# daihangpku/SW-NeRF

Hardware: AMD Instinct MI355X
Metric: rays/sec (64+128 samples/ray) (higher is better)
Workload: dtype f32

## Files before the change

### sw-nerf_amd/csrc/colour_kernels.hip

```cpp
#include <hip/hip_runtime.h>
#include "../../include/swnerf.h"
#include "swnerf_common.h"
#include "mlp_core.h"
#include "host_util.h"
#include "mlp_kernels.h"
#include "render_pass.h"

__global__ void __launch_bounds__(1024) colour_scan_kernel(ViewWs vw, int64_t n_rays) {
    __shared__ int part[16];
    const int tid = threadIdx.x, lane = tid & 63, wv = tid >> 6;
    const int64_t K = (n_rays + 1023) / 1024;
    const int64_t r0 = tid * K, r1 = r0 + K < n_rays ? r0 + K : n_rays;
    int* off = vw_off(vw);
    int* segray = vw_segray(vw, n_rays);
    int sum = 0;
    for (int64_t r = r0; r < r1; ++r) sum += off[r];
    int v = sum;
#pragma unroll
    for (int o = 1; o < 64; o <<= 1) { const int up = __shfl_up(v, o, 64); if (lane >= o) v += up; }
    if (lane == 63) part[wv] = v;
    __syncthreads();
    int below = v - sum, total = 0;
#pragma unroll
    for (int k = 0; k < 16; ++k) { if (k < wv) below += part[k]; total += part[k]; }
    for (int64_t r = r0; r < r1; ++r) {
        const int cnt = off[r];
        off[r] = below;
        for (int g = (below + 31) >> 5; 32 * g < below + cnt; ++g) segray[g] = (int)r;
        below += cnt;
    }
    if (tid == 0) off[n_rays] = total;
}

struct ColourDev {
    ViewWs vw;
    const float* ray_batch; int cols; int64_t n_rays;
    const float* b0; int nbias;
    const float* wvl;
};

__global__ void __launch_bounds__(256, 2) colour_rows_kernel(ColourDev P) {
    extern __shared__ __attribute__((aligned(16))) float lds_bias[];
    const int lane = threadIdx.x & 63, j = lane & 31, h = lane >> 5;
    const int wv = __builtin_amdgcn_readfirstlane(threadIdx.x >> 6);
    bias_to_lds(lds_bias, P.b0, P.nbias);
    const int* off = vw_off(P.vw);
    const int* segray = vw_segray(P.vw, P.n_rays);
    const int total = __builtin_amdgcn_readfirstlane(off[P.n_rays]);
    const int nseg = (total + 31) >> 5, nwaves = (int)gridDim.x * 4;
    int g = (int)blockIdx.x * 4 + wv;
    if (g >= nseg) return;
    WStream ws;
    ws_start(ws, P.wvl, lds_bias, lds_bias + P.nbias + wv * SW_RING * SW_STEP_FLOATS, lane);
    const float* rgb_tiles = ws.bias + (SW_DIR_BIAS_TILES + 64 + 8 + 1) * SW_BIAS_TILE_FLOATS;
    const float* hb_rgb = rgb_tiles - SW_BIAS_TILE_FLOATS;
    const int gs = vw_group_stride(P.vw);
#pragma nounroll
    for (; g < nseg; g += nwaves) {
        const int row = 32 * g + j;
        const bool valid = row < total;
        const int i = valid ? row : total - 1;
        const int rg = __builtin_amdgcn_readfirstlane(segray[g]);
        const int64_t rk = (int64_t)rg + j + 1;
        const int nxt = off[rk < P.n_rays ? rk : P.n_rays];
        int dr = 0;
#pragma unroll
        for (int k = 0; k < 32; ++k) dr += (__shfl(nxt, k, 32) <= i) ? 1 : 0;
        const int64_t ray = (int64_t)rg + dr;
        const int slot = i - off[ray];
        float* reg = vw_ray(P.vw, ray);
        const int s = vw_sample(P.vw, reg)[slot];
        const float* q = vw_row(P.vw, reg, slot, h);
        f32x16 in[8], demb, hv[4];
#pragma unroll
        for (int c = 0; c < 32; ++c) {
            const f32x4 v = *reinterpret_cast<const f32x4*>(q + (size_t)c * gs);
            in[c >> 2][4 * (c & 3) + 0] = v[0]; in[c >> 2][4 * (c & 3) + 1] = v[1];
            in[c >> 2][4 * (c & 3) + 2] = v[2]; in[c >> 2][4 * (c & 3) + 3] = v[3];
        }
        const float* dp = P.ray_batch + ray * P.cols + (P.cols - 3);
        pe_dir(dp[0], dp[1], dp[2], h, demb);
        ws.bias = rgb_tiles;
        ws.base = reinterpret_cast<const char*>(P.wvl);
        canon_tail_rows(in, demb, hv, lds_bias + h * 16, ws);
        float c3[3];
        head_valu<3, 4>(hv, ws, c3);
        if (valid && h == 0) {
            float* c = vw_c(P.vw, reg);
            c[s] = c3[0] + hb_rgb[1]; c[P.vw.sp + s] = c3[1] + hb_rgb[2]; c[2 * P.vw.sp + s] = c3[2] + hb_rgb[3];
        }
    }
}

__global__ void __launch_bounds__(256) colour_maps_kernel(ViewWs vw, int64_t n_rays, int S, int white, float* rgb_map) {
    const int lane = threadIdx.x & 63, j = lane & 31;
    const int64_t ray = (int64_t)blockIdx.x * 4 + (threadIdx.x >> 6);
    if (ray >= n_rays) return;
    float* reg = vw_ray(vw, ray);
    const float* wq = vw_w(vw, reg);
    const float* cq = vw_c(vw, reg);
    float pr = 0.f, pg = 0.f, pb = 0.f;
    const int ntiles = (S + 31) >> 5;
#pragma nounroll
    for (int t = 0; t < ntiles; ++t) {
        const int s = t * 32 + j;
        const int sc = s < S ? s : S - 1;
        const float w = s < S ? wq[sc] : 0.f;
        const float c0 = cq[sc], c1 = cq[vw.sp + sc], c2 = cq[2 * vw.sp + sc];
        comp_accumulate_colour(w, c0, c1, c2, pr, pg, pb);
    }
    pr = wave32_sum(pr); pg = wave32_sum(pg); pb = wave32_sum(pb);
    if (lane == 0) comp_write_rgb(pr, pg, pb, reg[0], white, ray, rgb_map);
}

int sw_colour_split_launch(const swnerf_pass_args& a, const ViewWs& vw, const float* b0, int nbias, const float* wvl, hipStream_t st) {
    hipLaunchKernelGGL(colour_scan_kernel, dim3(1), dim3(1024), 0, st, vw, a.n_rays);
    const int64_t rows_max = a.n_rays * (int64_t)(vw.rows < a.n_samples ? vw.rows : a.n_samples);
    const int64_t wgs = (rows_max + 127) / 128;
    if (wgs > 0) {
        ColourDev P;
        P.vw = vw; P.ray_batch = a.ray_batch; P.cols = a.cols; P.n_rays = a.n_rays; P.b0 = b0; P.nbias = nbias; P.wvl = wvl;
        const size_t lds = ((size_t)nbias + 4 * SW_RING * SW_STEP_FLOATS) * sizeof(float);
        hipLaunchKernelGGL(colour_rows_kernel, dim3((unsigned)(wgs < 512 ? wgs : 512)), dim3(256), lds, st, P);
    }
    hipLaunchKernelGGL(colour_maps_kernel, dim3((unsigned)((a.n_rays + 3) / 4)), dim3(256), 0, st, vw, a.n_rays, a.n_samples, a.white_bkgd, a.rgb_map);
    return sw_check(hipGetLastError(), "render_pass colour launch");
}
```

### sw-nerf_amd/csrc/render_pass.h

```cpp
#pragma once
#include <cstdlib>
#include "mlp_kernels.h"
#include "mlp_core_x3.h"
#include "resample.h"
#include "composite.h"
#include "ray_rows.h"

#define SW_LDS_SC 256
#define SW_LDS_SORT 1024
#define SW_LDS_WAVE_FLOATS (3 * SW_LDS_SC + SW_LDS_SORT)

#define SW_DEFER_SMAX 240
#define SW_DEFER_WS_FLOATS (64 * 256)
#define SW_DEFER_SEGS_PER_RAY ((SW_DEFER_SMAX + 31) / 32)

struct ViewWs {
    float* base;
    int64_t hdr, per_ray;
    int rows, sp;
};

static inline int64_t view_ws_hdr(int64_t n_rays) { return ((n_rays + 1 + 3) & ~(int64_t)3) + SW_DEFER_SEGS_PER_RAY * n_rays; }
static inline int64_t view_ws_full(int64_t n_rays, int S) {
    const int64_t sp = (S + 3) & ~3;
    return view_ws_hdr(n_rays) + n_rays * (4 + 4 * sp + 257 * sp);
}
static inline ViewWs view_ws_layout(float* base, int64_t floats, int64_t n_rays, int S) {
    ViewWs v = {};
    v.base = base;
    v.sp = (S + 3) & ~3;
    v.hdr = view_ws_hdr(n_rays);
    const int64_t avail = n_rays > 0 ? ((floats - v.hdr) / n_rays) & ~(int64_t)3 : 0;
    int64_t r = ((avail - 4 - 4 * v.sp) / 257) & ~(int64_t)3;
    if (r > v.sp) r = v.sp;
    v.rows = r > 0 ? (int)r : 0;
    v.per_ray = 4 + 4 * (int64_t)v.sp + 257 * (int64_t)v.rows;
    return v;
}
__device__ __forceinline__ int* vw_off(const ViewWs& v) { return reinterpret_cast<int*>(v.base); }
__device__ __forceinline__ int* vw_segray(const ViewWs& v, int64_t n_rays) { return reinterpret_cast<int*>(v.base) + ((n_rays + 1 + 3) & ~(int64_t)3); }
__device__ __forceinline__ float* vw_ray(const ViewWs& v, int64_t ray) { return v.base + v.hdr + ray * v.per_ray; }
__device__ __forceinline__ float* vw_w(const ViewWs& v, float* reg) { return reg + 4; }
__device__ __forceinline__ float* vw_c(const ViewWs& v, float* reg) { return reg + 4 + v.sp; }
__device__ __forceinline__ int* vw_sample(const ViewWs& v, float* reg) { return reinterpret_cast<int*>(reg + 4 + 4 * v.sp); }
__device__ __forceinline__ float* vw_row(const ViewWs& v, float* reg, int slot, int h) { return reg + 4 + 4 * v.sp + v.rows + (h * v.rows + slot) * 4; }
__device__ __forceinline__ int vw_group_stride(const ViewWs& v) { return 8 * v.rows; }

struct PassDev {
    swnerf_pass_args a;
    const float* w0;
    const float* b0;
    int nbias;
    int two_pass;
    int sort_n, sort_s;
    float* act;
    float* bits;
    float* xs;
    float* act_d; float* bits_d; float* xs_d;
    int dir_steps;
    int time_steps;
    int tb_off;
    int warm_steps;
    int warm_blocks;
    int skew_mode;
    int skew_unit;
    ViewWs vw;
};

__device__ __forceinline__ float wave32_sum(float v) {
#pragma unroll
    for (int o = 16; o > 0; o >>= 1) v += __shfl_xor(v, o, 32);
    return v;
}

__device__ __forceinline__ float z_linear(const swnerf_pass_args& a, float near, float far, int s) {
    const float t = sw_linspace(0.f, 1.f, a.n_samples, s);
    if (!a.lindisp) return near * (1.f - t) + far * t;
    return 1.f / (1.f / near * (1.f - t) + 1.f / far * t);
}

__device__ __forceinline__ float z_sample(const swnerf_pass_args& a, int64_t ray, float near, float far, int s) {
    const int S = a.n_samples;
    if (a.z_vals) return a.z_vals[ray * S + s];
    const float zs = z_linear(a, near, far, s);
    if (!a.t_rand) return zs;
    const float upper = (s < S - 1) ? .5f * (z_linear(a, near, far, s + 1) + zs) : zs;
    const float lower = (s > 0) ? .5f * (zs + z_linear(a, near, far, s - 1)) : zs;
    return lower + (upper - lower) * a.t_rand[ray * S + s];
}

#define SW_WARM_MAX_PER_WAVE 48
__device__ __forceinline__ void pass_startup(const PassDev& P, const float* w0, float* junk, int lane, int wv) {
    const unsigned b = blockIdx.x;
    if (P.warm_steps > 0 && (int)(b >> 3) < P.warm_blocks) {
        const unsigned junk_addr = __builtin_amdgcn_readfirstlane((unsigned)(size_t)junk);
        const int stride = P.warm_blocks * 4;
        int s = (int)(b >> 3) * 4 + wv;
#pragma nounroll
        for (int i = 0; i < SW_WARM_MAX_PER_WAVE && s < P.warm_steps; ++i, s += stride)
            ws_dma(reinterpret_cast<const char*>(w0) + (size_t)s * 1024, (unsigned)lane * 16u, junk_addr);
    }
    if (P.skew_mode) {
        const int k = (P.skew_mode == 1 ? (int)(b >> 3) : (int)(b >> 3) * 4 + wv) & 15;
#pragma nounroll
        for (int i = 0; i < k; ++i) __builtin_amdgcn_s_sleep(4);
        (void)P.skew_unit;
    }
}

static inline void pass_startup_args(PassDev& P, unsigned grid_x, int steps) {
    const char* ew = getenv("SWNERF_WARM");
    const char* es = getenv("SWNERF_SKEW");
    const int env_warm = ew ? atoi(ew) : 1, env_skew = es ? atoi(es) : 2;
    const unsigned first_round = grid_x < 256u ? grid_x : 256u;
    P.warm_blocks = (int)(first_round / 8u);
    P.warm_steps = (env_warm && P.warm_blocks > 0) ? steps + SW_TAIL : 0;
    P.skew_mode = env_skew;
    P.skew_unit = 4;
}

struct PassAccepts {
    const char* name;
    unsigned cols[4];
    int shape_code;
    const char* shape_msg;
    bool time_band;
    int smax;
};
#define SW_COLS(c) (1u << (c))

static inline int pass_check(const PassAccepts& e, const swnerf_pass_args& a) {
    if (!a.packed || (!a.ray_batch && a.n_rays != 0)) return sw_fail(SWNERF_E_ARG, e.smax ? "%s: NULL pointer" : "%s: NULL ray_batch/packed", e.name);
    if (a.kind < 0 || a.kind > 3 || a.cols < 0 || a.cols > 31 || !(e.cols[a.kind] >> a.cols & 1u)) return sw_fail(e.shape_code, e.shape_msg, e.name, a.cols, a.kind);
    if (e.smax && (a.n_rays < 0 || a.n_samples < 2 || a.n_samples > e.smax))
        return sw_fail(SWNERF_E_UNSUPP, "%s: 2 <= n_samples <= %d (got %d)", e.name, e.smax, a.n_samples);
    if (a.n_rays < 0 || a.n_samples < 2) return sw_fail(SWNERF_E_ARG, "%s: n_rays %lld, n_samples %d", e.name, (long long)a.n_rays, a.n_samples);
    if (a.L_pos < 0 || a.L_pos > 10 || a.L_dir < 0 || a.L_dir > 4 || (e.time_band && (a.L_time < 0 || a.L_time > 10)))
        return e.time_band ? sw_fail(SWNERF_E_UNSUPP, "%s: embedder bands (%d,%d,%d) exceed (10,4,10)", e.name, a.L_pos, a.L_dir, a.L_time)
                           : sw_fail(SWNERF_E_UNSUPP, "%s: embedder bands (%d,%d) exceed (10,4)", e.name, a.L_pos, a.L_dir);
    if (a.z_vals && a.t_rand) return sw_fail(SWNERF_E_ARG, "%s: t_rand only applies to coarse sampling", e.name);
    return 0;
}

static inline PassDev pass_dev(const swnerf_pass_args& a) {
    PassDev P = {};
    P.a = a;
    return P;
}

static inline int pass_resampling(const char* name, const swnerf_pass_args& a, PassDev& P, size_t& lds) {
    if (a.n_importance <= 0) return 0;
    if (!a.z_fine && a.n_rays != 0) return sw_fail(SWNERF_E_ARG, "%s: n_importance>0 needs z_fine", name);
    if (a.n_samples < 3 || a.n_samples > SW_LDS_SC || a.n_samples + a.n_importance > SW_LDS_SORT)
        return sw_fail(SWNERF_E_UNSUPP, "%s: resampling supports 3<=N_samples<=%d and N_samples+N_importance<=%d", name, SW_LDS_SC, SW_LDS_SORT);
    P.sort_n = P.sort_s = 2;
    while (P.sort_n < a.n_importance) P.sort_n <<= 1;
    while (P.sort_s < a.n_samples) P.sort_s <<= 1;
    lds += 4 * SW_LDS_WAVE_FLOATS * sizeof(float);
    return 0;
}

template <bool VEC4>
__device__ __forceinline__ void comp_bwd_ray(const float* raw, int oc, const float* zv, const float* noise, int S, int lane, float dnorm,
                                             int white, const float* g_rgb, const float* g_disp, const float* g_acc,
                                             float* T_, float* W_, float* dR) {
    CompGrads g = {g_rgb ? g_rgb[0] : 0.f, g_rgb ? g_rgb[1] : 0.f, g_rgb ? g_rgb[2] : 0.f, g_acc ? g_acc[0] : 0.f, 0.f, g_rgb != nullptr};
    double Tc = 1.0;
    float pa = 0.f, pd = 0.f;
    for (int base = 0; base < S; base += 64) {
        const int s = base + lane;
        const bool live = s < S;
        const int sc = live ? s : S - 1;
        const float z = zv[sc];
        const float zn = (s + 1 < S) ? zv[s + 1] : z;
        const float dist = comp_dist(s + 1 < S, zn, z, dnorm);
        float sg = raw[sc * oc + 3];
        if (noise) sg += noise[sc];
        const float alpha = comp_alpha(sg, dist, live);
        const float T = comp_transmittance(excl_cumprod_shfl<64>(comp_survival(alpha), lane), Tc);
        const float w = alpha * T;
        if (live) { T_[s] = T; W_[s] = w; }
        pa += w; pd += w * z;
    }
#pragma unroll
    for (int o = 32; o > 0; o >>= 1) { pa += __shfl_xor(pa, o, 64); pd += __shfl_xor(pd, o, 64); }
    comp_bwd_fold(g, white, g_disp, pd, pa);
    wave_lds_sync();
    double carry = 0.0;
    const int nch = (S + 63) / 64;
    for (int ch = nch - 1; ch >= 0; --ch) {
        const int s = ch * 64 + lane;
        const bool live = s < S;
        const int sc = live ? s : S - 1;
        f32x4 r4;
        if (!VEC4) { r4[0] = raw[sc * oc]; r4[1] = raw[sc * oc + 1]; r4[2] = raw[sc * oc + 2]; r4[3] = raw[sc * oc + 3]; }
        else r4 = *reinterpret_cast<const f32x4*>(raw + sc * 4);
        const float z = zv[sc];
        const float c0 = comp_sigmoid(r4[0]), c1 = comp_sigmoid(r4[1]), c2 = comp_sigmoid(r4[2]);
        const float w = live ? W_[sc] : 0.f, T = live ? T_[sc] : 0.f;
        const float G = comp_bwd_G(g, c0, c1, c2, z);
        double v = live ? (double)G * (double)w : 0.0;
#pragma unroll
        for (int o = 1; o < 64; o <<= 1) { const double dn = __shfl_down(v, o, 64); if (lane + o < 64) v += dn; }
        double after = __shfl_down(v, 1, 64);
        if (lane == 63) after = 0.0;
        const double R = carry + after;
        carry += __shfl(v, 0, 64);
        const float zn = (s + 1 < S) ? zv[s + 1] : z;
        const float dist = comp_dist(s + 1 < S, zn, z, dnorm);
        float sg = r4[3];
        if (noise) sg += noise[sc];
        const f32x4 o4 = comp_bwd_sample(g, G, T, w, R, sg, dist, c0, c1, c2);
        if (live) *reinterpret_cast<f32x4*>(dR + 4 * s) = o4;
    }
    wave_lds_sync();
}

template <bool DNERF, bool TRAIN> struct PassLds {
    static constexpr int TRAIN_TILES = SW_NOVIEW_BIAS_TILES(SW_NOVIEW_MAX_OUT) > SW_CANON_BIAS_TILES ? SW_NOVIEW_BIAS_TILES(SW_NOVIEW_MAX_OUT) : SW_CANON_BIAS_TILES;
    static constexpr int BIAS = (TRAIN && !DNERF) ? TRAIN_TILES * SW_BIAS_TILE_FLOATS : SW_LDS_BIAS_FLOATS;
    static constexpr int FIXED = BIAS + 4 * SW_LDS_RING_FLOATS;
};
template <bool DNERF> struct X3Lds {
    static constexpr int BIAS = (DNERF ? SW_DEFORM_BIAS_TILES + SW_X3_CANON_BIAS_TILES : SW_X3_CANON_BIAS_TILES) * SW_BIAS_TILE_FLOATS;
    static constexpr int DIR = DNERF ? 0 : 16 * 64;
    static constexpr int WAVE = DIR + SW_ZSLOT_FLOATS;
    static constexpr int FIXED = BIAS + X3_RING_FLOATS + 4 * WAVE;
};

template <bool DNERF, bool TRAIN = false, int PREC = 0, bool VIEWS = true>
__global__ void __launch_bounds__(256, 1) render_pass_kernel(PassDev P) {
    static_assert(PREC == 0 || !TRAIN, "the bf16 paths cover the inference passes");
    static_assert(VIEWS || (!DNERF && PREC == 0), "the no-view-direction variant is a static fp32 pass (inference or TRAIN)");
    extern __shared__ __attribute__((aligned(16))) float lds_all[];
    const swnerf_pass_args& a = P.a;
    const int lane = threadIdx.x & 63, j = lane & 31, h = lane >> 5;
    const int wv = __builtin_amdgcn_readfirstlane(threadIdx.x >> 6);
    const int64_t ray_id = (int64_t)blockIdx.x * 4 + wv;
    if constexpr (PREC == 0)
        pass_startup(P, P.w0, lds_all + PassLds<DNERF, TRAIN>::BIAS + wv * SW_LDS_RING_FLOATS + SW_RING * SW_STEP_FLOATS, lane, wv);
    bias_to_lds(lds_all, P.b0, P.nbias);
    const bool ghost = PREC != 0 && ray_id >= a.n_rays;
    if (PREC == 0 && ray_id >= a.n_rays) return;
    const int64_t ray = ghost ? a.n_rays - 1 : ray_id;
    const float* lds_bias = lds_all;
    float* lds_ring = PREC ? lds_all + X3Lds<DNERF>::BIAS
                           : lds_all + PassLds<DNERF, TRAIN>::BIAS + wv * SW_LDS_RING_FLOATS;
    float* lds_emb = lds_ring + SW_RING * SW_STEP_FLOATS;
    float* lds_x3w = lds_ring + X3_RING_FLOATS + wv * X3Lds<DNERF>::WAVE;
    float* lds_dir = PREC ? lds_x3w : lds_emb + 2 * 16 * 64;
    float* lds_vb = lds_emb + SW_EMB_LDS_FLOATS + SW_ZSLOT_FLOATS;
    const float* lds_tb = (DNERF && PREC == 0 && P.time_steps) ? lds_all + P.tb_off + wv * SW_TB_LDS_FLOATS : nullptr;
    float* lds = PREC ? lds_all + X3Lds<DNERF>::FIXED + wv * SW_LDS_WAVE_FLOATS
                      : lds_all + PassLds<DNERF, TRAIN>::FIXED + wv * SW_LDS_WAVE_FLOATS;
    float* zc = lds;
    float* wc = lds + SW_LDS_SC;
    float* cdf = lds + 2 * SW_LDS_SC;
    float* srt = lds + 3 * SW_LDS_SC;

    const int S = a.n_samples;
    const bool resample = a.n_importance > 0;
    const float* rb = a.ray_batch + ray * a.cols;
    const float ox = rb[0], oy = rb[1], oz = rb[2], dx = rb[3], dy = rb[4], dz = rb[5];
    const float near = rb[6], far = rb[7];
    const float ft = (a.cols == 12) ? rb[8] : 0.f;
    const float v0 = VIEWS ? rb[a.cols - 3] : 0.f, v1 = VIEWS ? rb[a.cols - 2] : 0.f, v2 = VIEWS ? rb[a.cols - 1] : 0.f;
    const float dnorm = row_dnorm(ox, oy, oz, dx, dy, dz, near, far, ft);

    WStream ws;
    XStream xs;
    if constexpr (PREC != 0) {
        if (!DNERF) {
            f32x16 demb;
            pe_dir(v0, v1, v2, h, demb);
            tile_park(lds_dir, lane, demb);
        }
        x3_start(xs, reinterpret_cast<const char*>(P.w0), lds_bias, lds_ring, lane, wv);
    } else {
        ws_start(ws, P.w0, lds_bias, lds_ring, lane);
        if constexpr (VIEWS) {
            f32x16 demb;
            pe_dir(v0, v1, v2, h, demb);
            if constexpr (TRAIN) tile_park(lds_dir, lane, demb);
            view_bias_tile(demb, lds_vb, lane, ws);
        }
        if constexpr (DNERF) {
            if (P.time_steps) time_bias_tile(ft, h, lds_all + P.tb_off + wv * SW_TB_LDS_FLOATS, lane, ws);
        }
    }

    const float* zrow = a.z_vals ? a.z_vals + ray * S : nullptr;
    const float* zslot = PREC ? lds_x3w + X3Lds<DNERF>::DIR : lds_emb + SW_EMB_LDS_FLOATS;
    const unsigned zslot_addr = __builtin_amdgcn_readfirstlane((unsigned)(size_t)zslot);
    float pr = 0.f, pg = 0.f, pb = 0.f, pd = 0.f, pa = 0.f;
    double Tc = 1.0;
    const int ntiles = (S + 31) >> 5;
    constexpr bool DEFER_OK = !DNERF && !TRAIN && PREC == 0 && VIEWS;
    const bool defer = DEFER_OK && P.vw.base != nullptr;
    float* vreg = defer ? vw_ray(P.vw, ray) : nullptr;
    const char* main_head = reinterpret_cast<const char*>(P.w0 + (P.dir_steps + P.time_steps) * SW_STEP_FLOATS);
    int wr = 0;
#pragma nounroll
    for (int tile = 0; tile < ntiles; ++tile) {
        const bool stash = defer && wr + min(32, S - tile * 32) <= P.vw.rows;
        const int s = tile * 32 + j;
        const bool live = s < S && !ghost;
        const int sc = live ? s : S - 1;
        float z, zn;
        if (zrow && tile > 0) {
            const float* zs = zslot + (tile & 1) * 64;
            z = zs[j];
            const float z1 = zs[j + 1];
            zn = (s + 1 < S) ? z1 : z;
        } else {
            z = z_sample(a, ray, near, far, sc);
            zn = (s + 1 < S) ? z_sample(a, ray, near, far, s + 1) : z;
        }
        if (zrow && tile + 1 < ntiles)
            lds_dma_dword(reinterpret_cast<const char*>(zrow), (unsigned)min(32 * (tile + 1) + lane, S - 1) * 4u,
                          zslot_addr + (unsigned)((tile + 1) & 1) * 256u);
        float px = ox + dx * z, py = oy + dy * z, pz = oz + dz * z;

        f32x16 emb[2], in[8], out[8];
        float head[3], rgb[3];
        float extra = 0.f;
        pe_pos(px, py, pz, h, emb);
        if (DNERF && TRAIN) {
            const int64_t tix = ray * ntiles + tile, prow = tix * 32 + j;
            float* act_row = P.act + prow * SW_ACT_LD + 4 * h;
            float* mask_tile = P.bits + tix * SW_MASK_TILE_FLOATS + lane * 4;
            float* xs_row = P.xs + prow * SW_XS_LD + 4 * h;
            f32x4 mb = {0.f, 0.f, 0.f, 0.f};
            f32x16 demb;
#pragma nounroll
            for (int pass = 0; pass < 2; ++pass) {
                const bool dp = pass == 0;
                trunk_pass<true, true, true, false, true>(emb, lds_emb, ft, dp, h, in, out, head, ws,
                                             dp ? P.act_d + prow * SW_ACT_LD + 4 * h : act_row,
                                             dp ? P.bits_d + tix * SW_MASK_TILE_FLOATS + lane * 4 : mask_tile, dp, &mb,
                                             dp ? P.xs_d + prow * SW_XS_LD + 4 * h : xs_row, lds_tb);
                if (dp) {
                    const float ex = head[0], ey = head[1], ez = head[2];
                    if (live && h == 0) {
                        float* o = a.dx + (ray * S + s) * 3;
                        o[0] = ex; o[1] = ey; o[2] = ez;
                    }
                    px = px + ex; py = py + ey; pz = pz + ez;
                    pe_pos(px, py, pz, h, emb);
                    tile_fetch(lds_dir, lane, demb);
#pragma unroll
                    for (int g = 0; g < 4; ++g) {
                        const f32x4 v = {demb[4 * g], demb[4 * g + 1], demb[4 * g + 2], demb[4 * g + 3]};
                        *reinterpret_cast<f32x4*>(xs_row + 64 + 8 * g) = v;
                    }
                }
            }
            canon_tail_train(in, lds_vb, rgb, ws.bias - SW_BIAS_TILE_FLOATS, ws, act_row, mask_tile, mb);
        } else if (DNERF && PREC != 0) {
            if constexpr (DNERF && PREC != 0) {
#pragma nounroll
                for (int pass = P.two_pass ? 0 : 1; pass < 2; ++pass) {
                    x3_net_dn_pipe<PREC>(px, py, pz, ft, pass == 0, h, v0, v1, v2, head, rgb, xs);
                    if (pass == 0) {
                        const float ex = head[0], ey = head[1], ez = head[2];
                        if (a.dx && live && h == 0) {
                            float* o = a.dx + (ray * S + s) * 3;
                            o[0] = ex; o[1] = ey; o[2] = ez;
                        }
                        px = px + ex; py = py + ey; pz = pz + ez;
                    }
                }
                if (!P.two_pass && a.dx && live && h == 0) {
                    float* o = a.dx + (ray * S + s) * 3;
                    o[0] = 0.f; o[1] = 0.f; o[2] = 0.f;
                }
                x3_rewind(xs, P.two_pass ? SW_X3_DEFORM_CHUNKS + SW_X3_CANON_CHUNKS : SW_X3_CANON_CHUNKS, lds_bias, lane);
            }
        } else if (DNERF) {
#pragma nounroll
            for (int pass = P.two_pass ? 0 : 1; pass < 2; ++pass) {
                trunk_pass<true, false, false, false, true>(emb, lds_emb, ft, pass == 0, h, in, out, head, ws, nullptr, nullptr, false, nullptr, nullptr, lds_tb);
                if (pass == 0) {
                    const float ex = head[0], ey = head[1], ez = head[2];
                    if (a.dx && live && h == 0) {
                        float* o = a.dx + (ray * S + s) * 3;
                        o[0] = ex; o[1] = ey; o[2] = ez;
                    }
                    px = px + ex; py = py + ey; pz = pz + ez;
                    pe_pos(px, py, pz, h, emb);
                }
            }
            if (!P.two_pass && a.dx && live && h == 0) {
                float* o = a.dx + (ray * S + s) * 3;
                o[0] = 0.f; o[1] = 0.f; o[2] = 0.f;
            }
        } else if (TRAIN && !VIEWS) {
            const int64_t prow = (ray * ntiles + tile) * 32 + j;
            float* act_row = P.act + prow * SW_ACT_LD + 4 * h;
            float* mask_tile = P.bits + (ray * ntiles + tile) * SW_MASK_TILE_FLOATS + lane * 4;
            float* xs_row = P.xs + prow * SW_XS_LD + 4 * h;
            f32x4 mb = {0.f, 0.f, 0.f, 0.f};
            trunk_pass<false, true, true, true>(emb, lds_emb, 0.f, false, h, in, out, head, ws, act_row, mask_tile, true, &mb, xs_row);
            float o5[5] = {0.f, 0.f, 0.f, 0.f, 0.f};
            head_valu_rt<8>(in, ws, a.out_ch, o5);
            rgb[0] = o5[0] + ws.bias[0]; rgb[1] = o5[1] + ws.bias[1]; rgb[2] = o5[2] + ws.bias[2];
            head[0] = o5[3] + ws.bias[3]; head[1] = 0.f; head[2] = 0.f;
            extra = o5[4] + ws.bias[4];
        } else if (TRAIN) {
            const int64_t prow = (ray * ntiles + tile) * 32 + j;
            float* act_row = P.act + prow * SW_ACT_LD + 4 * h;
            float* mask_tile = P.bits + (ray * ntiles + tile) * SW_MASK_TILE_FLOATS + lane * 4;
            float* xs_row = P.xs + prow * SW_XS_LD + 4 * h;
            f32x4 mb = {0.f, 0.f, 0.f, 0.f};
            f32x16 demb;
            tile_fetch(lds_dir, lane, demb);
#pragma unroll
            for (int g = 0; g < 4; ++g) {
                const f32x4 v = {demb[4 * g], demb[4 * g + 1], demb[4 * g + 2], demb[4 * g + 3]};
                *reinterpret_cast<f32x4*>(xs_row + 64 + 8 * g) = v;
            }
            trunk_pass<false, true, true>(emb, lds_emb, 0.f, false, h, in, out, head, ws, act_row, mask_tile, false, &mb, xs_row);
            canon_tail_train(in, lds_vb, rgb, ws.bias - SW_BIAS_TILE_FLOATS, ws, act_row, mask_tile, mb);
        } else if constexpr (PREC != 0) {
            head[1] = 0.f; head[2] = 0.f;
            x3_canon_pipe<PREC>(px, py, pz, h, lds_dir, lane, head[0], rgb, xs);
            x3_rewind(xs, SW_X3_CANON_CHUNKS, lds_bias, lane);
        } else if constexpr (!VIEWS) {
            trunk_pass<false, false, false, true>(emb, lds_emb, 0.f, false, h, in, out, head, ws);
            float o5[5] = {0.f, 0.f, 0.f, 0.f, 0.f};
            const int nout = (a.out_ch == 5 && !a.raw) ? 4 : a.out_ch;
            head_valu_rt<8>(in, ws, nout, o5);
            ws.bias += (a.out_ch - nout) * 8 * SW_BIAS_TILE_FLOATS;
            rgb[0] = o5[0] + ws.bias[0]; rgb[1] = o5[1] + ws.bias[1]; rgb[2] = o5[2] + ws.bias[2];
            head[0] = o5[3] + ws.bias[3]; head[1] = 0.f; head[2] = 0.f;
            extra = o5[4] + ws.bias[4];
        } else {
            trunk_pass<false, false, false, false, false, true>(emb, lds_emb, 0.f, false, h, in, out, head, ws, nullptr, nullptr, false,
                                                                nullptr, nullptr, nullptr, stash ? main_head : nullptr);
        }

        const float sg_raw = head[0];
        float sg = sg_raw;
        if (a.noise) sg += a.noise[ray * S + sc];
        const float alpha = comp_alpha(sg, comp_dist(s + 1 < S, zn, z, dnorm), live);
        const float w = alpha * comp_transmittance(excl_cumprod_shfl<32>(comp_survival(alpha), j), Tc);
        if (live) {
            if (a.weights && h == 0) a.weights[ray * S + s] = w;
            if (a.z_out && h == 0) a.z_out[ray * S + s] = z;
            if (resample && h == 0) { zc[s] = z; wc[s] = w; }
        }
        comp_accumulate_density(w, z, pd, pa);

        bool lit = live;
        if constexpr (DEFER_OK) {
            if (defer) {
                lit = live && (!(alpha == 0.f) || s == 0);
                if (live && h == 0) vw_w(P.vw, vreg)[s] = w;
                if (stash) {
                    const unsigned m = (unsigned)__ballot(lit);
                    const int slot = wr + __popc(m & ((1u << j) - 1u));
                    if (lit) {
                        if (h == 0) vw_sample(P.vw, vreg)[slot] = s;
                        float* q = vw_row(P.vw, vreg, slot, h);
                        const int gs = vw_group_stride(P.vw);
#pragma unroll
                        for (int c = 0; c < 32; ++c) {
                            const f32x4 v = {in[c >> 2][4 * (c & 3)], in[c >> 2][4 * (c & 3) + 1], in[c >> 2][4 * (c & 3) + 2], in[c >> 2][4 * (c & 3) + 3]};
                            *reinterpret_cast<f32x4*>(q + (size_t)c * gs) = v;
                        }
                    }
                    wr += __builtin_amdgcn_readfirstlane(__popc(m));
                }
            }
        }
        if (!TRAIN && PREC == 0 && VIEWS) {
            if (!stash) {
                if constexpr (DEFER_OK) ws.cont = ws.base + SW_STEPS_VIEWSH * 1024;
                canon_tail<DEFER_OK>(in, lds_vb, rgb, ws.bias - SW_BIAS_TILE_FLOATS, ws);
            } else {
                rgb[0] = 0.f; rgb[1] = 0.f; rgb[2] = 0.f;
            }
        }
        if constexpr (PREC == 0) {
            ws_rewind(ws, P.w0 + (P.dir_steps + P.time_steps) * SW_STEP_FLOATS,
                      lds_bias + ((P.dir_steps ? SW_DIR_BIAS_TILES : 0) + (P.time_steps ? 8 : 0)) * SW_BIAS_TILE_FLOATS, lane);
        }

        const float c0 = rgb[0], c1 = rgb[1], c2 = rgb[2];
        if (DEFER_OK && defer) {
            if (live && h == 0) {
                float* c = vw_c(P.vw, vreg);
                const bool here = lit && !stash;
                c[s] = here ? c0 : 0.f; c[P.vw.sp + s] = here ? c1 : 0.f; c[2 * P.vw.sp + s] = here ? c2 : 0.f;
            }
            continue;
        }
        if (a.raw && live && h == 0) {
            if (!VIEWS && a.out_ch == 5) {
                float* o = a.raw + (ray * S + s) * 5;
                o[0] = c0; o[1] = c1; o[2] = c2; o[3] = sg_raw; o[4] = extra;
            } else {
                f32x4 r4 = {c0, c1, c2, sg_raw};
                *reinterpret_cast<f32x4*>(a.raw + (ray * S + s) * 4) = r4;
            }
        }
        comp_accumulate_colour(w, c0, c1, c2, pr, pg, pb);
    }

    pr = wave32_sum(pr); pg = wave32_sum(pg); pb = wave32_sum(pb);
    pd = wave32_sum(pd); pa = wave32_sum(pa);
    if (lane == 0 && !ghost) comp_write_maps(pr, pg, pb, pd, pa, a.white_bkgd, ray, defer ? nullptr : a.rgb_map, a.disp_map, a.acc_map, a.depth_map);
    if constexpr (DEFER_OK) {
        if (defer && lane == 0) { vw_off(P.vw)[ray] = wr; vreg[0] = pa; }
    }
    if (!resample || ghost) return;

    wave_lds_sync();
    const int Ni = a.n_importance;
    const double sm = wave_sample_pdf(wc + 1, S - 1, MidBins{zc}, a.u ? a.u + ray * Ni : nullptr, Ni, cdf, srt, lane);
    if (a.z_std) {
        const float sd = wave_zstd(sm, srt, Ni, lane);
        if (lane == 0) a.z_std[ray] = sd;
    }
    wave_rank_merge(zc, S, P.sort_s, srt, Ni, P.sort_n, a.z_fine + ray * (S + Ni), lane);
}
```

Baseline: 562,200.

## Parallelize colour scan, prefetch next segment lookup, skip unused dir bias

Above a ray-count threshold, the single-workgroup prefix scan over per-ray row counts is replaced with a two-kernel multi-block scan that stores block sums in spare segray space. The colour rows kernel now software-pipelines its segment-to-ray lookup, loading the next segment's offset window and segray entry during the current MLP work and pinning the load order with sched barriers. Separately, the main render pass skips the view-direction bias tile when the deferred colour pass covers all samples. This adds an extra kernel launch and more register pressure from the prefetch state, and depends on the spare segray space being large enough.

Result: no change. 565,600 (median of 6 runs) (+0.6%).

```diff
diff --git a/sw-nerf_amd/csrc/colour_kernels.hip b/sw-nerf_amd/csrc/colour_kernels.hip
--- a/sw-nerf_amd/csrc/colour_kernels.hip
+++ b/sw-nerf_amd/csrc/colour_kernels.hip
@@ -1,10 +1,12 @@
 #include <hip/hip_runtime.h>
+#include <cstdlib>
 #include "../../include/swnerf.h"
 #include "swnerf_common.h"
 #include "mlp_core.h"
 #include "host_util.h"
 #include "mlp_kernels.h"
 #include "render_pass.h"
+#include "par_prims.h"
 
 __global__ void __launch_bounds__(1024) colour_scan_kernel(ViewWs vw, int64_t n_rays) {
     __shared__ int part[16];
@@ -32,6 +34,43 @@
     if (tid == 0) off[n_rays] = total;
 }
 
+#define SW_SCAN_BLOCK 1024
+__device__ __forceinline__ int* vw_scan_sums(const ViewWs& v, int64_t n_rays, int nblk) { return vw_segray(v, n_rays) + SW_DEFER_SEGS_PER_RAY * n_rays - nblk; }
+
+__global__ void __launch_bounds__(SW_SCAN_BLOCK) colour_scan_sums_kernel(ViewWs vw, int64_t n_rays) {
+    __shared__ int part[SW_SCAN_BLOCK / 64];
+    const int64_t r = (int64_t)blockIdx.x * SW_SCAN_BLOCK + threadIdx.x;
+    const int cnt = r < n_rays ? vw_off(vw)[r] : 0;
+    int sum;
+    block_exclusive_scan<int, SW_SCAN_BLOCK>(cnt, part, &sum);
+    if (threadIdx.x == 0) vw_scan_sums(vw, n_rays, (int)gridDim.x)[blockIdx.x] = sum;
+}
+
+__global__ void __launch_bounds__(SW_SCAN_BLOCK) colour_scan_wide_kernel(ViewWs vw, int64_t n_rays) {
+    __shared__ int part[SW_SCAN_BLOCK / 64];
+    const int tid = threadIdx.x, b = (int)blockIdx.x, nblk = (int)gridDim.x;
+    const int* sums = vw_scan_sums(vw, n_rays, nblk);
+    int lo = 0, all = 0;
+    for (int k = tid; k < nblk; k += SW_SCAN_BLOCK) {
+        const int v = sums[k];
+        all += v;
+        if (k < b) lo += v;
+    }
+    int base, total, mine;
+    block_exclusive_scan<int, SW_SCAN_BLOCK>(lo, part, &base);
+    block_exclusive_scan<int, SW_SCAN_BLOCK>(all, part, &total);
+    int* off = vw_off(vw);
+    int* segray = vw_segray(vw, n_rays);
+    const int64_t r = (int64_t)b * SW_SCAN_BLOCK + tid;
+    const int cnt = r < n_rays ? off[r] : 0;
+    const int below = base + block_exclusive_scan<int, SW_SCAN_BLOCK>(cnt, part, &mine);
+    if (r < n_rays) {
+        off[r] = below;
+        for (int g = (below + 31) >> 5; 32 * g < below + cnt; ++g) segray[g] = (int)r;
+    }
+    if (b == 0 && tid == 0) off[n_rays] = total;
+}
+
 struct ColourDev {
     ViewWs vw;
     const float* ray_batch; int cols; int64_t n_rays;
@@ -39,17 +78,47 @@
     const float* wvl;
 };
 
+__device__ __forceinline__ int colour_ray_clamp(int r, int64_t n_rays) { return r < 0 ? 0 : (r < n_rays ? r : (int)(n_rays - 1)); }
+
+__device__ __forceinline__ int colour_window(const int* off, int rg, int lane, int64_t n_rays) {
+    const int64_t rk = (int64_t)rg + lane;
+    return off[rk < n_rays ? rk : n_rays];
+}
+
+__device__ __forceinline__ void colour_locate(int win, int rg, int g, int j, int total, bool& valid, int64_t& ray, int& slot) {
+    const int row = 32 * g + j;
+    valid = row < total;
+    const int i = valid ? row : total - 1;
+    int dr = 0;
+#pragma unroll
+    for (int k = 0; k < 32; ++k) dr += (__builtin_amdgcn_readlane(win, k + 1) <= i) ? 1 : 0;
+    ray = (int64_t)rg + dr;
+    slot = i - __shfl(win, dr, 64);
+}
+
 __global__ void __launch_bounds__(256, 2) colour_rows_kernel(ColourDev P) {
     extern __shared__ __attribute__((aligned(16))) float lds_bias[];
     const int lane = threadIdx.x & 63, j = lane & 31, h = lane >> 5;
     const int wv = __builtin_amdgcn_readfirstlane(threadIdx.x >> 6);
-    bias_to_lds(lds_bias, P.b0, P.nbias);
     const int* off = vw_off(P.vw);
     const int* segray = vw_segray(P.vw, P.n_rays);
-    const int total = __builtin_amdgcn_readfirstlane(off[P.n_rays]);
-    const int nseg = (total + 31) >> 5, nwaves = (int)gridDim.x * 4;
+    const int nwaves = (int)gridDim.x * 4;
     int g = (int)blockIdx.x * 4 + wv;
+    const int64_t segcap = (int64_t)SW_DEFER_SEGS_PER_RAY * P.n_rays;
+    const int total_v = off[P.n_rays];
+    const int rg_v = segray[g < segcap ? g : segcap - 1];
+    const int rgn_v = segray[(int64_t)g + nwaves < segcap ? (int64_t)g + nwaves : segcap - 1];
+    const int rg = colour_ray_clamp(__builtin_amdgcn_readfirstlane(rg_v), P.n_rays);
+    int rgn = colour_ray_clamp(__builtin_amdgcn_readfirstlane(rgn_v), P.n_rays);
+    const int win = colour_window(off, rg, lane, P.n_rays);
+    bias_to_lds(lds_bias, P.b0, P.nbias);
+    const int total = __builtin_amdgcn_readfirstlane(total_v);
+    const int nseg = (total + 31) >> 5;
     if (g >= nseg) return;
+    bool valid;
+    int64_t ray;
+    int slot;
+    colour_locate(win, rg, g, j, total, valid, ray, slot);
     WStream ws;
     ws_start(ws, P.wvl, lds_bias, lds_bias + P.nbias + wv * SW_RING * SW_STEP_FLOATS, lane);
     const float* rgb_tiles = ws.bias + (SW_DIR_BIAS_TILES + 64 + 8 + 1) * SW_BIAS_TILE_FLOATS;
@@ -57,20 +126,15 @@
     const int gs = vw_group_stride(P.vw);
 #pragma nounroll
     for (; g < nseg; g += nwaves) {
-        const int row = 32 * g + j;
-        const bool valid = row < total;
-        const int i = valid ? row : total - 1;
-        const int rg = __builtin_amdgcn_readfirstlane(segray[g]);
-        const int64_t rk = (int64_t)rg + j + 1;
-        const int nxt = off[rk < P.n_rays ? rk : P.n_rays];
-        int dr = 0;
-#pragma unroll
-        for (int k = 0; k < 32; ++k) dr += (__shfl(nxt, k, 32) <= i) ? 1 : 0;
-        const int64_t ray = (int64_t)rg + dr;
-        const int slot = i - off[ray];
         float* reg = vw_ray(P.vw, ray);
+        const float* q = vw_row(P.vw, reg, slot, h);
+        const int gnn = g + 2 * nwaves < nseg ? g + 2 * nwaves : g;
+        const int rgnn_v = segray[gnn];
+        const int win_n = colour_window(off, rgn, lane, P.n_rays);
         const int s = vw_sample(P.vw, reg)[slot];
-        const float* q = vw_row(P.vw, reg, slot, h);
+        const float* dp = P.ray_batch + ray * P.cols + (P.cols - 3);
+        const float d0 = dp[0], d1 = dp[1], d2 = dp[2];
+        __builtin_amdgcn_sched_barrier(0);
         f32x16 in[8], demb, hv[4];
 #pragma unroll
         for (int c = 0; c < 32; ++c) {
@@ -78,17 +142,19 @@
             in[c >> 2][4 * (c & 3) + 0] = v[0]; in[c >> 2][4 * (c & 3) + 1] = v[1];
             in[c >> 2][4 * (c & 3) + 2] = v[2]; in[c >> 2][4 * (c & 3) + 3] = v[3];
         }
-        const float* dp = P.ray_batch + ray * P.cols + (P.cols - 3);
-        pe_dir(dp[0], dp[1], dp[2], h, demb);
+        __builtin_amdgcn_sched_barrier(0);
+        pe_dir(d0, d1, d2, h, demb);
+        const int rgnn = __builtin_amdgcn_readfirstlane(rgnn_v);
         ws.bias = rgb_tiles;
         ws.base = reinterpret_cast<const char*>(P.wvl);
         canon_tail_rows(in, demb, hv, lds_bias + h * 16, ws);
         float c3[3];
         head_valu<3, 4>(hv, ws, c3);
-        if (valid && h == 0) {
-            float* c = vw_c(P.vw, reg);
-            c[s] = c3[0] + hb_rgb[1]; c[P.vw.sp + s] = c3[1] + hb_rgb[2]; c[2 * P.vw.sp + s] = c3[2] + hb_rgb[3];
-        }
+        float* c = vw_c(P.vw, reg);
+        const bool store = valid && h == 0;
+        colour_locate(win_n, rgn, g + nwaves, j, total, valid, ray, slot);
+        rgn = rgnn;
+        if (store) { c[s] = c3[0] + hb_rgb[1]; c[P.vw.sp + s] = c3[1] + hb_rgb[2]; c[2 * P.vw.sp + s] = c3[2] + hb_rgb[3]; }
     }
 }
 
@@ -113,8 +179,19 @@
     if (lane == 0) comp_write_rgb(pr, pg, pb, reg[0], white, ray, rgb_map);
 }
 
+#define SW_SCAN_WIDE_RAYS 16384
+
 int sw_colour_split_launch(const swnerf_pass_args& a, const ViewWs& vw, const float* b0, int nbias, const float* wvl, hipStream_t st) {
-    hipLaunchKernelGGL(colour_scan_kernel, dim3(1), dim3(1024), 0, st, vw, a.n_rays);
+    const char* es = getenv("SWNERF_SCAN_WIDE");
+    const int64_t wide_from = es ? atoll(es) : SW_SCAN_WIDE_RAYS;
+    const int64_t nblk = (a.n_rays + SW_SCAN_BLOCK - 1) / SW_SCAN_BLOCK;
+    const bool sums_fit = (a.n_rays * SW_DEFER_SMAX + 31) / 32 + nblk <= (int64_t)SW_DEFER_SEGS_PER_RAY * a.n_rays;
+    if (a.n_rays >= wide_from && sums_fit) {
+        hipLaunchKernelGGL(colour_scan_sums_kernel, dim3((unsigned)nblk), dim3(SW_SCAN_BLOCK), 0, st, vw, a.n_rays);
+        hipLaunchKernelGGL(colour_scan_wide_kernel, dim3((unsigned)nblk), dim3(SW_SCAN_BLOCK), 0, st, vw, a.n_rays);
+    } else {
+        hipLaunchKernelGGL(colour_scan_kernel, dim3(1), dim3(1024), 0, st, vw, a.n_rays);
+    }
     const int64_t rows_max = a.n_rays * (int64_t)(vw.rows < a.n_samples ? vw.rows : a.n_samples);
     const int64_t wgs = (rows_max + 127) / 128;
     if (wgs > 0) {
diff --git a/sw-nerf_amd/csrc/render_pass.h b/sw-nerf_amd/csrc/render_pass.h
--- a/sw-nerf_amd/csrc/render_pass.h
+++ b/sw-nerf_amd/csrc/render_pass.h
@@ -277,12 +277,16 @@
         }
         x3_start(xs, reinterpret_cast<const char*>(P.w0), lds_bias, lds_ring, lane, wv);
     } else {
-        ws_start(ws, P.w0, lds_bias, lds_ring, lane);
+        const bool no_dir = !DNERF && !TRAIN && VIEWS && P.vw.base != nullptr && P.vw.rows >= a.n_samples;
+        ws_start(ws, no_dir ? P.w0 + P.dir_steps * SW_STEP_FLOATS : P.w0,
+                 no_dir ? lds_bias + SW_DIR_BIAS_TILES * SW_BIAS_TILE_FLOATS : lds_bias, lds_ring, lane);
         if constexpr (VIEWS) {
-            f32x16 demb;
-            pe_dir(v0, v1, v2, h, demb);
-            if constexpr (TRAIN) tile_park(lds_dir, lane, demb);
-            view_bias_tile(demb, lds_vb, lane, ws);
+            if (!no_dir) {
+                f32x16 demb;
+                pe_dir(v0, v1, v2, h, demb);
+                if constexpr (TRAIN) tile_park(lds_dir, lane, demb);
+                view_bias_tile(demb, lds_vb, lane, ws);
+            }
         }
         if constexpr (DNERF) {
             if (P.time_steps) time_bias_tile(ft, h, lds_all + P.tb_off + wv * SW_TB_LDS_FLOATS, lane, ws);
```

## Parallelize colour scan, prefetch segment windows, skip unused view-dir bias in deferred pass

Applied to the files above, without the earlier changes.

Above a ray-count threshold, the single-workgroup prefix scan is replaced by a three-kernel multi-block scan: per-block sums, scan of block bases, then fill. The colour rows kernel now prefetches the next segment's ray window and segray entry one iteration ahead, resolves ray and slot offsets from a register window with readlane and shfl, and overlaps weight priming with bias loading. In the deferred render pass, the view-direction bias tile computation and its weight steps are skipped when the colour work is deferred to the split kernel. These changes add launches and register pressure, and the no_dir predicate must correctly match the cases that actually defer.

Result: no change. 562,800 before, 564,200 after (median of 6 runs) (+0.3%).

```diff
diff --git a/sw-nerf_amd/csrc/colour_kernels.hip b/sw-nerf_amd/csrc/colour_kernels.hip
--- a/sw-nerf_amd/csrc/colour_kernels.hip
+++ b/sw-nerf_amd/csrc/colour_kernels.hip
@@ -6,30 +6,90 @@
 #include "mlp_kernels.h"
 #include "render_pass.h"
 
-__global__ void __launch_bounds__(1024) colour_scan_kernel(ViewWs vw, int64_t n_rays) {
-    __shared__ int part[16];
-    const int tid = threadIdx.x, lane = tid & 63, wv = tid >> 6;
-    const int64_t K = (n_rays + 1023) / 1024;
-    const int64_t r0 = tid * K, r1 = r0 + K < n_rays ? r0 + K : n_rays;
-    int* off = vw_off(vw);
-    int* segray = vw_segray(vw, n_rays);
-    int sum = 0;
-    for (int64_t r = r0; r < r1; ++r) sum += off[r];
+
+__device__ __forceinline__ void scan_1024(int sum, int* part, int& below, int& total) {
+    const int lane = threadIdx.x & 63, wv = threadIdx.x >> 6;
     int v = sum;
 #pragma unroll
     for (int o = 1; o < 64; o <<= 1) { const int up = __shfl_up(v, o, 64); if (lane >= o) v += up; }
     if (lane == 63) part[wv] = v;
     __syncthreads();
-    int below = v - sum, total = 0;
+    below = v - sum; total = 0;
 #pragma unroll
     for (int k = 0; k < 16; ++k) { if (k < wv) below += part[k]; total += part[k]; }
+}
+
+__device__ __forceinline__ void scan_fill(int* off, int* segray, int64_t r0, int64_t r1, int below) {
     for (int64_t r = r0; r < r1; ++r) {
         const int cnt = off[r];
         off[r] = below;
         for (int g = (below + 31) >> 5; 32 * g < below + cnt; ++g) segray[g] = (int)r;
         below += cnt;
     }
+}
+
+__global__ void __launch_bounds__(1024) colour_scan_kernel(ViewWs vw, int64_t n_rays) {
+    __shared__ int part[16];
+    const int tid = threadIdx.x;
+    const int64_t K = (n_rays + 1023) / 1024;
+    const int64_t r0 = tid * K, r1 = r0 + K < n_rays ? r0 + K : n_rays;
+    int* off = vw_off(vw);
+    int sum = 0;
+    for (int64_t r = r0; r < r1; ++r) sum += off[r];
+    int below, total;
+    scan_1024(sum, part, below, total);
+    scan_fill(off, vw_segray(vw, n_rays), r0, r1, below);
     if (tid == 0) off[n_rays] = total;
+}
+
+__device__ __forceinline__ void wide_span(int64_t n_rays, int br, int64_t& r0, int64_t& r1) {
+    const int64_t K = (br + 1023) / 1024;
+    const int64_t lo = (int64_t)blockIdx.x * br, hi = lo + br < n_rays ? lo + br : n_rays;
+    r0 = lo + threadIdx.x * K < hi ? lo + threadIdx.x * K : hi;
+    r1 = r0 + K < hi ? r0 + K : hi;
+}
+__device__ __forceinline__ int* wide_cell(const ViewWs& vw, int64_t b, int br) { return reinterpret_cast<int*>(vw_ray(vw, b * br) + 1); }
+
+__global__ void __launch_bounds__(1024) colour_scan_sums_kernel(ViewWs vw, int64_t n_rays, int br) {
+    __shared__ int part[16];
+    int64_t r0, r1;
+    wide_span(n_rays, br, r0, r1);
+    const int* off = vw_off(vw);
+    int sum = 0;
+    for (int64_t r = r0; r < r1; ++r) sum += off[r];
+    int below, total;
+    scan_1024(sum, part, below, total);
+    if (threadIdx.x == 0) *wide_cell(vw, blockIdx.x, br) = total;
+}
+
+__global__ void __launch_bounds__(1024) colour_scan_bases_kernel(ViewWs vw, int64_t n_rays, int br, int64_t nb) {
+    __shared__ int part[16];
+    const int tid = threadIdx.x;
+    const int64_t K = (nb + 1023) / 1024;
+    const int64_t b0 = tid * K < nb ? tid * K : nb, b1 = b0 + K < nb ? b0 + K : nb;
+    int sum = 0;
+    for (int64_t b = b0; b < b1; ++b) sum += *wide_cell(vw, b, br);
+    int below, total;
+    scan_1024(sum, part, below, total);
+    for (int64_t b = b0; b < b1; ++b) {
+        int* cell = wide_cell(vw, b, br);
+        const int cnt = *cell;
+        *cell = below;
+        below += cnt;
+    }
+    if (tid == 0) vw_off(vw)[n_rays] = total;
+}
+
+__global__ void __launch_bounds__(1024) colour_scan_fill_kernel(ViewWs vw, int64_t n_rays, int br) {
+    __shared__ int part[16];
+    int64_t r0, r1;
+    wide_span(n_rays, br, r0, r1);
+    int* off = vw_off(vw);
+    int sum = 0;
+    for (int64_t r = r0; r < r1; ++r) sum += off[r];
+    int below, total;
+    scan_1024(sum, part, below, total);
+    scan_fill(off, vw_segray(vw, n_rays), r0, r1, *wide_cell(vw, blockIdx.x, br) + below);
 }
 
 struct ColourDev {
@@ -39,35 +99,62 @@
     const float* wvl;
 };
 
+__device__ __forceinline__ int seg_window(const int* off, int rg, int lane, int64_t n_rays) {
+    const int64_t k = (int64_t)rg + lane;
+    return off[k < n_rays ? k : n_rays];
+}
+
 __global__ void __launch_bounds__(256, 2) colour_rows_kernel(ColourDev P) {
     extern __shared__ __attribute__((aligned(16))) float lds_bias[];
     const int lane = threadIdx.x & 63, j = lane & 31, h = lane >> 5;
     const int wv = __builtin_amdgcn_readfirstlane(threadIdx.x >> 6);
-    bias_to_lds(lds_bias, P.b0, P.nbias);
     const int* off = vw_off(P.vw);
     const int* segray = vw_segray(P.vw, P.n_rays);
-    const int total = __builtin_amdgcn_readfirstlane(off[P.n_rays]);
-    const int nseg = (total + 31) >> 5, nwaves = (int)gridDim.x * 4;
+    const int nwaves = (int)gridDim.x * 4;
     int g = (int)blockIdx.x * 4 + wv;
+    WStream ws;
+    ws.base = reinterpret_cast<const char*>(P.wvl);
+    ws.voff = (unsigned)lane * 16u;
+    ws.lds_addr = __builtin_amdgcn_readfirstlane((unsigned)(size_t)(lds_bias + P.nbias + wv * SW_RING * SW_STEP_FLOATS));
+    ws.ring = lds_bias + P.nbias + wv * SW_RING * SW_STEP_FLOATS + lane * 4;
+    ws.bias = lds_bias + h * 16;
+    ws.cont = nullptr;
+    ws_prime<0>(ws);
+    const int64_t g0 = g < SW_DEFER_SEGS_PER_RAY * P.n_rays ? g : 0;
+    const int total_v = off[P.n_rays], rg_v = segray[g0];
+    const int total = __builtin_amdgcn_readfirstlane(total_v);
+    const int nseg = (total + 31) >> 5;
+    int rg = g < nseg ? __builtin_amdgcn_readfirstlane(rg_v) : 0;
+    int win = 0, rgn_v = 0;
+    if (g < nseg) {
+        win = seg_window(off, rg, lane, P.n_rays);
+        if (g + nwaves < nseg) rgn_v = segray[g + nwaves];
+    }
+    bias_to_lds(lds_bias, P.b0, P.nbias);
+    ws_wait<0>();
     if (g >= nseg) return;
-    WStream ws;
-    ws_start(ws, P.wvl, lds_bias, lds_bias + P.nbias + wv * SW_RING * SW_STEP_FLOATS, lane);
+    ws.a_cur = ws_read(ws, 0);
     const float* rgb_tiles = ws.bias + (SW_DIR_BIAS_TILES + 64 + 8 + 1) * SW_BIAS_TILE_FLOATS;
     const float* hb_rgb = rgb_tiles - SW_BIAS_TILE_FLOATS;
     const int gs = vw_group_stride(P.vw);
 #pragma nounroll
     for (; g < nseg; g += nwaves) {
+        const int gn = g + nwaves;
+        const int rgn = __builtin_amdgcn_readfirstlane(rgn_v);
+        int win_n = 0;
+        rgn_v = 0;
+        if (gn < nseg) {
+            win_n = seg_window(off, rgn, lane, P.n_rays);
+            if (gn + nwaves < nseg) rgn_v = segray[gn + nwaves];
+        }
         const int row = 32 * g + j;
         const bool valid = row < total;
         const int i = valid ? row : total - 1;
-        const int rg = __builtin_amdgcn_readfirstlane(segray[g]);
-        const int64_t rk = (int64_t)rg + j + 1;
-        const int nxt = off[rk < P.n_rays ? rk : P.n_rays];
         int dr = 0;
 #pragma unroll
-        for (int k = 0; k < 32; ++k) dr += (__shfl(nxt, k, 32) <= i) ? 1 : 0;
+        for (int k = 1; k <= 32; ++k) dr += (__builtin_amdgcn_readlane(win, k) <= i) ? 1 : 0;
         const int64_t ray = (int64_t)rg + dr;
-        const int slot = i - off[ray];
+        const int slot = i - __shfl(win, dr, 64);
         float* reg = vw_ray(P.vw, ray);
         const int s = vw_sample(P.vw, reg)[slot];
         const float* q = vw_row(P.vw, reg, slot, h);
@@ -89,6 +176,7 @@
             float* c = vw_c(P.vw, reg);
             c[s] = c3[0] + hb_rgb[1]; c[P.vw.sp + s] = c3[1] + hb_rgb[2]; c[2 * P.vw.sp + s] = c3[2] + hb_rgb[3];
         }
+        rg = rgn; win = win_n;
     }
 }
 
@@ -113,15 +201,34 @@
     if (lane == 0) comp_write_rgb(pr, pg, pb, reg[0], white, ray, rgb_map);
 }
 
+#define SW_SCAN_WIDE_RAYS 8192
+#define SW_SCAN_WG_RAYS 4096
+#define SW_COLOUR_WGS 512
+static inline int64_t env_or(const char* name, int64_t dflt, int64_t lo, int64_t hi) {
+    const char* e = getenv(name);
+    if (!e || !*e) return dflt;
+    const long long v = atoll(e);
+    return v < lo ? lo : (v > hi ? hi : (int64_t)v);
+}
+
 int sw_colour_split_launch(const swnerf_pass_args& a, const ViewWs& vw, const float* b0, int nbias, const float* wvl, hipStream_t st) {
-    hipLaunchKernelGGL(colour_scan_kernel, dim3(1), dim3(1024), 0, st, vw, a.n_rays);
+    if (a.n_rays <= env_or("SWNERF_SCAN_WIDE_RAYS", SW_SCAN_WIDE_RAYS, 0, INT64_MAX)) {
+        hipLaunchKernelGGL(colour_scan_kernel, dim3(1), dim3(1024), 0, st, vw, a.n_rays);
+    } else {
+        const int br = (int)env_or("SWNERF_SCAN_WG_RAYS", SW_SCAN_WG_RAYS, 1, 1 << 20);
+        const int64_t nb = (a.n_rays + br - 1) / br;
+        hipLaunchKernelGGL(colour_scan_sums_kernel, dim3((unsigned)nb), dim3(1024), 0, st, vw, a.n_rays, br);
+        hipLaunchKernelGGL(colour_scan_bases_kernel, dim3(1), dim3(1024), 0, st, vw, a.n_rays, br, nb);
+        hipLaunchKernelGGL(colour_scan_fill_kernel, dim3((unsigned)nb), dim3(1024), 0, st, vw, a.n_rays, br);
+    }
     const int64_t rows_max = a.n_rays * (int64_t)(vw.rows < a.n_samples ? vw.rows : a.n_samples);
     const int64_t wgs = (rows_max + 127) / 128;
     if (wgs > 0) {
         ColourDev P;
         P.vw = vw; P.ray_batch = a.ray_batch; P.cols = a.cols; P.n_rays = a.n_rays; P.b0 = b0; P.nbias = nbias; P.wvl = wvl;
         const size_t lds = ((size_t)nbias + 4 * SW_RING * SW_STEP_FLOATS) * sizeof(float);
-        hipLaunchKernelGGL(colour_rows_kernel, dim3((unsigned)(wgs < 512 ? wgs : 512)), dim3(256), lds, st, P);
+        const int64_t cap = env_or("SWNERF_COLOUR_WGS", SW_COLOUR_WGS, 1, SW_COLOUR_WGS);
+        hipLaunchKernelGGL(colour_rows_kernel, dim3((unsigned)(wgs < cap ? wgs : cap)), dim3(256), lds, st, P);
     }
     hipLaunchKernelGGL(colour_maps_kernel, dim3((unsigned)((a.n_rays + 3) / 4)), dim3(256), 0, st, vw, a.n_rays, a.n_samples, a.white_bkgd, a.rgb_map);
     return sw_check(hipGetLastError(), "render_pass colour launch");
diff --git a/sw-nerf_amd/csrc/render_pass.h b/sw-nerf_amd/csrc/render_pass.h
--- a/sw-nerf_amd/csrc/render_pass.h
+++ b/sw-nerf_amd/csrc/render_pass.h
@@ -277,12 +277,16 @@
         }
         x3_start(xs, reinterpret_cast<const char*>(P.w0), lds_bias, lds_ring, lane, wv);
     } else {
-        ws_start(ws, P.w0, lds_bias, lds_ring, lane);
+        const bool no_dir = !DNERF && !TRAIN && VIEWS && P.vw.base != nullptr && P.vw.sp <= P.vw.rows;
+        ws_start(ws, no_dir ? P.w0 + P.dir_steps * SW_STEP_FLOATS : P.w0,
+                 no_dir ? lds_bias + (P.dir_steps ? SW_DIR_BIAS_TILES : 0) * SW_BIAS_TILE_FLOATS : lds_bias, lds_ring, lane);
         if constexpr (VIEWS) {
-            f32x16 demb;
-            pe_dir(v0, v1, v2, h, demb);
-            if constexpr (TRAIN) tile_park(lds_dir, lane, demb);
-            view_bias_tile(demb, lds_vb, lane, ws);
+            if (!no_dir) {
+                f32x16 demb;
+                pe_dir(v0, v1, v2, h, demb);
+                if constexpr (TRAIN) tile_park(lds_dir, lane, demb);
+                view_bias_tile(demb, lds_vb, lane, ws);
+            }
         }
         if constexpr (DNERF) {
             if (P.time_steps) time_bias_tile(ft, h, lds_all + P.tb_off + wv * SW_TB_LDS_FLOATS, lane, ws);
```
